# Black-Phoenix/CUDA-SfM

Measured on AMD Instinct MI355X. Metric: RANSAC E-matrix hypotheses/sec (8-point, fused scoring), inlier-mask parity vs CPU oracle, higher is better.
Workload: dtype f32

## Files before the change

cuda-sfm_amd/csrc/prefilter_lds.hpp:

```cpp
#pragma once
#include "prefilter_record.hpp"

namespace sfm {

constexpr int kPfTileMax = 1024;
constexpr int kPfWaves = 16;
constexpr int kPfRing = 128;

constexpr int kPfERow = 10;
constexpr int kPfWaveBytes = 32 * kPfERow * 4 + 32 * 4;
template <int RULE> struct PfLds {
    static constexpr int kFragsPerBlock = RULE == kPfRuleG ? 3 : 2;
    static constexpr int kBlockBytes = kFragsPerBlock * 64 * 16;
    static constexpr int kFrag = 0;
    static constexpr int kTileMax = kPfTileMax;
    int staged, pts, ring, wave, next, lut, bytes;
    __host__ __device__ explicit PfLds(int tile, int ring_entries = kPfRing, int entry_bytes = 8)
    {
        staged = (tile + 63) & ~63;
        pts = kFrag + (staged / 32) * kBlockBytes;
        ring = pts + staged * 16;
        ring = (ring + ring_entries * entry_bytes - 1) & ~(ring_entries * entry_bytes - 1);
        wave = ring + kPfWaves * ring_entries * entry_bytes;
        next = wave + kPfWaves * kPfWaveBytes;
        lut = next + 16;
        bytes = lut + 32;
    }
};
static_assert(kPfRing * 8 == 1024, "ring slots are addressed with (offset & 1023) | base");

static inline int pf_tile_points(int ld, int tmax)
{
    const int ntiles = (ld + tmax - 1) / tmax;
    const int t = ((ld + ntiles - 1) / ntiles + 31) & ~31;
    return t < 32 ? 32 : t;
}

constexpr unsigned long long kPfSumCountsMin = 1ull << 21;
static inline bool pf_sums_counts_at(unsigned count, int ld, int tile)
{
    return (unsigned long long)count * (unsigned long long)((ld + tile - 1) / tile) >= kPfSumCountsMin;
}

}
```

cuda-sfm_amd/csrc/prefilter_record.hpp:

```cpp
#pragma once
#include "prefilter_math.hpp"

namespace sfm {

typedef _Float16 h8 __attribute__((ext_vector_type(8)));

constexpr int kPfRuleG = 0, kPfRuleBand = 1, kPfRuleBandPack = 2, kPfRuleBandTile = 3;
constexpr uint32_t kPfTileFlagScan = 1u;
constexpr uint32_t kPfTileFlagBSafe = 2u;
constexpr int kPfGroup = 32;
constexpr unsigned short kPfFlagScan = 0x3C00u;

struct alignas(16) PfRecord {
    unsigned short lo[16];
    unsigned short hi[16];
};
static_assert(sizeof(PfRecord) == 64, "4 x 16 bytes per hypothesis");

#if defined(__HIPCC__)
__device__ __forceinline__ uint32_t pf_cells_slot(uint32_t key, uint32_t mask) { return (key >> 7) & mask; }

__device__ __forceinline__ void pf_prep_store(const float e[9], float thr, float B, const PfScales &sc, const uint32_t *__restrict__ cells,
                                              uint32_t cells_mask, PfRecord *out)
{
// ... 115 lines not shown
__device__ __forceinline__ uint32_t pf_tile_flags(const float e[9], float B, const uint32_t *__restrict__ cells, uint32_t cells_mask);
__device__ __forceinline__ uint4 pf_tile_record(const float e[9], float B, const uint32_t *__restrict__ cells, uint32_t cells_mask)
{
    float dn, lin;
    prefilter_band_hyp_terms(e, B, dn, lin);
    return make_uint4(pf_tile_flags(e, B, cells, cells_mask), __float_as_uint(dn), __float_as_uint(lin), 0u);
}

__device__ __forceinline__ uint32_t pf_tile_flags(const float e[9], float B, const uint32_t *__restrict__ cells, uint32_t cells_mask)
{
    const PfGrid grid = prefilter_grid(B);
    int cx0, cx1, cy0, cy1;
    const int zs = prefilter_zero_divisor_cells(e, B, grid, cx0, cx1, cy0, cy1);
    bool scan = zs == 2;
    if (zs == 1) scan = !cells || pf_cells_occupied(cells, cells_mask, cx0, cx1, cy0, cy1, 0);
    float et[9];
    prefilter_transposed(e, et);
    const int zb = prefilter_zero_divisor_cells(et, B, grid, cx0, cx1, cy0, cy1);
    bool b_safe = zb == 0;
    if (zb == 1) b_safe = cells && !pf_cells_occupied(cells, cells_mask, cx0, cx1, cy0, cy1, 1);
    return (scan ? kPfTileFlagScan : 0u) | (b_safe ? kPfTileFlagBSafe : 0u);
}

__device__ __forceinline__ void pf_tile_operands(const float e[9], uint32_t flags, float dn, float lin, float thr, float B, const PfBox &box, int half, h8 &n0, h8 &n1)
{
    const float d_mine = prefilter_band_divisor_max(e, lin, box, half);
    const float d_other = __shfl_xor(d_mine, 32);
    const float sigma = prefilter_band_sigma_from_maxima(dn, thr, B, half ? d_other : d_mine, half ? d_mine : d_other, (flags & kPfTileFlagBSafe) != 0u, kPfBandTopPack);
    _Float16 ns[kPfSlots];
    prefilter_band_hyp_slots(e, sigma, ns);
#pragma unroll
    for (int j = 0; j < 8; ++j) { n0[j] = half ? ns[8 + j] : ns[j]; n1[j] = half ? ns[24 + j] : ns[16 + j]; }
}

__device__ __forceinline__ void pf_band_record_expand(const uint4 r0, const uint4 r1, int half, h8 &n0, h8 &n1, uint32_t &flag)
{
    uint32_t o[8];
    if (half == 0) {
        const uint32_t A0 = r0.x, A1 = r0.y, A2 = r0.z, A3 = r0.w, A4 = r1.x, A5 = r1.y;
        o[0] = pf_pick(A0, 0, A0, 0); o[1] = pf_pick(A0, 1, A1, 0); o[2] = A1;                  o[3] = pf_pick(A2, 0, A2, 0);
        o[4] = pf_pick(A2, 1, A3, 0); o[5] = pf_pick(A3, 1, A3, 1); o[6] = A4;                  o[7] = pf_pick(A4, 1, A5, 0);
        flag = 0u;
    } else {
        const uint32_t B0 = r0.x, B1 = r0.y, B2 = r0.z, B3 = r0.w, B4 = r1.x;
        o[0] = B0;                  o[1] = pf_pick(B0, 1, B1, 0); o[2] = pf_pick(B1, 1, B1, 1); o[3] = B2;
        o[4] = B3;                  o[5] = (B4 & 0xFFFFu) | 0x3C000000u; o[6] = 0u;              o[7] = 0u;
        flag = B4 >> 16;
    }
    n0 = __builtin_bit_cast(h8, uint4{ o[0], o[1], o[2], o[3] });
    n1 = __builtin_bit_cast(h8, uint4{ o[4], o[5], o[6], o[7] });
}
#endif

}
```

cuda-sfm_amd/csrc/ransac_prefilter.hip:

```cpp
#include "ransac_device.hpp"
#include "block_ops.hpp"
#include "prefilter_math.hpp"
#include "prefilter_record.hpp"
#include "prefilter_lds.hpp"

namespace sfm {

typedef float f16v __attribute__((ext_vector_type(16)));


__device__ constexpr int kPfESlot[9] = { 2, 6, 1, 3, 5, 7, 0, 4, 8 };
__device__ __forceinline__ uint32_t shift_in_reject(uint32_t rejected, float nt, float G)
{
    return __builtin_amdgcn_alignbit(rejected, __float_as_uint(fmaf(-nt, nt, G)), 31);
}

__device__ __forceinline__ uint32_t scan16(const f16v &nt, const f16v &G)
{
    uint32_t rejected = 0u;
#pragma unroll
    for (int r = 0; r < 16; ++r) rejected = shift_in_reject(rejected, nt[r], G[r]);
    return rejected;
}

// ... 74 lines not shown

#define PF_SCHED_STEP()                                                 \
    do {                                                                \
        if (RULE != kPfRuleG) {                                         \
            __builtin_amdgcn_sched_group_barrier(0x008, 1, 0);          \
            __builtin_amdgcn_sched_group_barrier(0x002, 8, 0);          \
            __builtin_amdgcn_sched_group_barrier(0x008, 1, 0);          \
            __builtin_amdgcn_sched_group_barrier(0x002, 8, 0);          \
        } else {                                                        \
            __builtin_amdgcn_sched_group_barrier(0x008, 1, 0);          \
            __builtin_amdgcn_sched_group_barrier(0x002, 11, 0);         \
            __builtin_amdgcn_sched_group_barrier(0x008, 1, 0);          \
            __builtin_amdgcn_sched_group_barrier(0x002, 11, 0);         \
            __builtin_amdgcn_sched_group_barrier(0x008, 1, 0);          \
            __builtin_amdgcn_sched_group_barrier(0x002, 11, 0);         \
        }                                                               \
    } while (0)

constexpr int kPfVarTickets = 1;
constexpr int kPfVarDrainLocal = 2;
constexpr int kPfVarClosedDecode = 4;
constexpr int kPfVarAnswerEpilogue = 8;
constexpr int kPfVarDrainK1 = 16, kPfVarDrainK7 = 32;

constexpr int pf_score_waves_per_simd(int var, int rule, int fl2, int pipe, int wide, int prio)
{
    return ((var & kPfVarTickets) == 0 && (rule == kPfRuleBandTile || rule == kPfRuleBandPack) && !fl2 && !pipe && !wide && !prio) ? 5 : 4;
}

template <int W, int VAR = 0, int RULE = kPfRuleBandTile, int FL2 = 0, int PIPE = 0, int WIDE = 0, int PRIO = 0>
__global__ __launch_bounds__(W * 64, pf_score_waves_per_simd(VAR, RULE, FL2, PIPE, WIDE, PRIO))
void ransac_score_prefilter(const float *__restrict__ X0, const float *__restrict__ X1, int ld, int n,
                            const float *__restrict__ Ecand, const PfRecord *__restrict__ recs, uint32_t h0, uint32_t count, float thr,
                            int dynamic, int tile,
                            int *__restrict__ counts, uint32_t *__restrict__ tick,
                            unsigned long long *best_key, unsigned long long *best_key2, unsigned long long *__restrict__ clk,
                            const unsigned long long *__restrict__ bound_word, const uint32_t *__restrict__ tile_boxes)
{
    extern __shared__ __attribute__((aligned(16))) unsigned char smem[];
    const int lane = threadIdx.x & 63;
    const int wave = __builtin_amdgcn_readfirstlane(threadIdx.x >> 6);
    const bool probe = clk && blockIdx.x == 0 && blockIdx.y == 0 && threadIdx.x == 0;
    unsigned long long c0 = 0, w0 = 0;
    if (clk && blockIdx.x == 0 && blockIdx.y == 0 && wave == 0) { c0 = clock64(); w0 = wall_clock64(); }
#if SFM_AB
    const uint32_t trace_blk = blockIdx.y * gridDim.x + blockIdx.x;
    unsigned long long *trace = (clk && trace_blk < (uint32_t)kTraceBlocks) ? clk + 8 + (size_t)trace_blk * kTraceWords : nullptr;
    if (trace && threadIdx.x == 0) {
        trace[0] = wall_clock64();
        trace[2] = ((unsigned long long)__builtin_amdgcn_s_getreg((20 << 0) | (0 << 6) | (31 << 11)) << 32) |
                   (unsigned long long)__builtin_amdgcn_s_getreg((4 << 0) | (0 << 6) | (31 << 11));
        trace[3] = ((unsigned long long)blockIdx.y << 32) | blockIdx.x;
    }
#define PF_PHASE(k) do { if (probe1) clk[k] = wall_clock64() - w0; } while (0)
#else
#define PF_PHASE(k) do { } while (0)
#endif
    const int half = lane >> 5, row = lane & 31;
    const uint32_t npass = (count + (uint32_t)kPfGroup - 1u) / (uint32_t)kPfGroup;
    const uint32_t nstatic = gridDim.x * (uint32_t)W;
    using LT = PfLds<RULE>;
    constexpr bool kBand = RULE != kPfRuleG, kTile = RULE == kPfRuleBandTile, kPack = RULE == kPfRuleBandPack || kTile;
    static_assert(!(FL2 && kPack) && !((VAR & kPfVarTickets) && kPack), "the recorded variants were built on the v_alignbit scan");
    constexpr bool kTail9 = kPack && W == 16 && !FL2 && !PIPE && !WIDE && !PRIO && !(VAR & kPfVarTickets);
    static_assert(kTail9 || (VAR & ~kPfVarTickets) == 0, "the pass-tail switches belong to the product's two rules");
    constexpr int kDrainMore = !kTail9 ? 0 : (VAR & kPfVarDrainK1) ? 1 : (VAR & kPfVarDrainK7) ? 7 : (VAR & kPfVarDrainLocal) ? 3 : 0;
    constexpr bool kDecodeTable = !(kTail9 && (VAR & kPfVarClosedDecode));
    constexpr bool kSumCounts = kTail9 && !(VAR & kPfVarAnswerEpilogue);
    constexpr int kRing = FL2 ? 256 : kPfRing;
    constexpr int kEnt = WIDE ? 16 : 8;
    static_assert(!WIDE || (kPack && !PIPE && !FL2), "wide entries: the packed scan's plain loop only");
    const LT L(tile, kRing, kEnt);
    float *etab = reinterpret_cast<float *>(smem + L.wave + wave * kPfWaveBytes);
    int *cnt = reinterpret_cast<int *>(etab + 32 * kPfERow);

    PfFrags afrag = {};
    uint32_t key0 = 0u;
    float rec_dn = 0.0f, rec_lin = 0.0f;
    float e_row[9] = {};
    auto fetch_pass = [&](uint32_t pass, PfFrags &af, uint32_t &k0, float (&e)[9], float &dn, float &lin) {
        const uint32_t hf = pass * (uint32_t)kPfGroup;
        const uint32_t h = hf + (uint32_t)min(row, (int)min((uint32_t)kPfGroup, count - hf) - 1);
        if (kTile) {
            const float *src = Ecand + 9 * (size_t)h;
#pragma unroll
            for (int k = 0; k < 9; ++k) e[k] = src[k];
            const uint4 rec = reinterpret_cast<const uint4 *>(recs)[h];
            k0 = rec.x; dn = __uint_as_float(rec.y); lin = __uint_as_float(rec.z);
            return;
        }
        const uint4 *r = reinterpret_cast<const uint4 *>(recs + h) + 2 * half;
        const uint4 r0 = r[0], r1 = r[1];
        if (kBand) pf_band_record_expand(r0, r1, half, af.n0, af.n1, k0);
        else pf_record_expand(r0, r1, half, af.n0, af.n1, af.t, k0);
        if (half == 0) {
            const float *src = Ecand + 9 * (size_t)h;
#pragma unroll
            for (int k = 0; k < 9; ++k) e[k] = src[k];
        }
    };
    auto install_rows = [&](const float (&e)[9]) {
        if (half == 0) {
#pragma unroll
            for (int k = 0; k < 9; ++k) etab[32 * k + row] = e[kPfESlot[k]];
            cnt[row] = 0;
        }
    };
    uint32_t ps = blockIdx.x * (uint32_t)W + (uint32_t)wave;
    bool have = ps < npass;
    if (have) { fetch_pass(ps, afrag, key0, e_row, rec_dn, rec_lin); install_rows(e_row); }

    SFM_PHASE("stage_tile");
    uint32_t *next_idx = reinterpret_cast<uint32_t *>(smem + L.next);
    if (threadIdx.x == 0) *next_idx = (uint32_t)W;
    if (kPack && kDecodeTable && threadIdx.x < 32) smem[L.lut + threadIdx.x] = (unsigned char)pf_pack_code((int)threadIdx.x);
    float pf_B = 0.0f;
    uint32_t bw[8] = {};
    uint32_t bw_lane = 0u;
    if (kTile) {
        pf_B = __uint_as_float((uint32_t)(__hip_atomic_load(reinterpret_cast<const uint32_t *>(bound_word), __ATOMIC_RELAXED, __HIP_MEMORY_SCOPE_AGENT)));
        bw_lane = __hip_atomic_load(tile_boxes + 8 * blockIdx.y + (lane & 7), __ATOMIC_RELAXED, __HIP_MEMORY_SCOPE_AGENT);
    }
    __syncthreads();
    const int tile_first = blockIdx.y * tile;
    for (int t = threadIdx.x; t < L.staged; t += W * 64) {
        const int p = tile_first + t;
        float u = 0.f, v = 0.f, x = 0.f, y = 0.f;
        const bool real = p < n && t < tile;
// ... 14 lines not shown
#pragma unroll
            for (int hh = 0; hh < 2; ++hh) {
                h8 c;
#pragma unroll
                for (int j = 0; j < 8; ++j) c[j] = bn[ks * 16 + hh * 8 + j];
                *reinterpret_cast<h8 *>(blk + ks * 1024 + (hh * 32 + col) * 16) = c;
            }
        if (RULE == kPfRuleG) {
#pragma unroll
            for (int hh = 0; hh < 2; ++hh) {
                h8 c;
#pragma unroll
                for (int j = 0; j < 8; ++j) c[j] = bt[hh * 8 + j];
                *reinterpret_cast<h8 *>(blk + 2048 + (hh * 32 + col) * 16) = c;
            }
        }
    }
    __syncthreads();
    PfBox tbox = {};
    auto build_operands = [&](const float (&e)[9], uint32_t fl, float dn, float lin) {
        int half_l = half;
        float thr_l = thr, B_l = pf_B;
        asm volatile("" : "+v"(half_l), "+s"(thr_l), "+s"(B_l));
        pf_tile_operands(e, fl, dn, lin, thr_l, B_l, tbox, half_l, afrag.n0, afrag.n1);
        key0 = fl & kPfTileFlagScan;
    };
    if (kTile) {
#pragma unroll
        for (int k = 0; k < 8; ++k) bw[k] = (uint32_t)__builtin_amdgcn_readlane((int)bw_lane, k);
        pf_B = uniform(pf_B);
        tbox = pf_box_from_bits(bw, pf_B);
        tbox = PfBox{ uniform(tbox.xlo), uniform(tbox.xhi), uniform(tbox.ylo), uniform(tbox.yhi), uniform(tbox.ulo), uniform(tbox.uhi), uniform(tbox.vlo), uniform(tbox.vhi) };
        if (have) build_operands(e_row, key0, rec_dn, rec_lin);
    }
#if SFM_AB
    if (probe) clk[2] = wall_clock64() - w0;
#endif
    const int npb = (min(tile, ld - tile_first) + 31) >> 5;
    const int npp = (npb + 1) >> 1;
    const float4 *pts = reinterpret_cast<const float4 *>(smem + L.pts);
    lds_cf *etab_l = (lds_cf *)etab;
    lds_i *cnt_l = (lds_i *)cnt;
    lds_cu8 *lut_l = (lds_cu8 *)(smem + L.lut);
    const uint32_t ring_base = (uint32_t)(size_t)(__attribute__((address_space(3))) unsigned char *)(smem + L.ring) + (uint32_t)wave * (uint32_t)(kRing * kEnt);
    uint32_t ring_mask = (uint32_t)(kRing * kEnt - 1);
    asm("" : "+v"(ring_mask));
    auto ring_at = [&](uint32_t index8) {
        return (lds_u2 *)((__attribute__((address_space(3))) unsigned char *)0 + ((index8 & ring_mask) | ring_base));
    };
    auto ring_at16 = [&](uint32_t index16) {
        return (lds_u4 *)((__attribute__((address_space(3))) unsigned char *)0 + ((index16 & ring_mask) | ring_base));
    };
    lds_ch8 *frag_lane = (lds_ch8 *)(smem + LT::kFrag) + lane;
    const ThrBand band = make_band(thr);
    uint32_t passes_done = 0;

    while (have) {
        SFM_PHASE("pass_begin");
        const uint32_t h_first = ps * (uint32_t)kPfGroup;
        const int nvalid = (int)min((uint32_t)kPfGroup, count - h_first);
#if SFM_AB
        const bool probe1 = probe && passes_done == 0u;
#endif
        uint32_t ps_next = ps + nstatic;
        if (dynamic) {
            uint32_t got = 0u;
            if (lane == 0) got = atomicAdd(next_idx, 1u);
            got = (uint32_t)__builtin_amdgcn_readfirstlane((int)got);
            ps_next = (got / (uint32_t)W) * nstatic + blockIdx.x * (uint32_t)W + (got % (uint32_t)W);
        }
        {
            const bool scan = key0 != 0u;
            const unsigned long long sm = __ballot(scan);
            uint32_t todo = (uint32_t)sm | (uint32_t)(sm >> 32);
            uint32_t survive = 0u;
            while (todo) {
                const int r = __builtin_ctz(todo);
                todo &= todo - 1u;
                const float se[6] = { etab[6 * 32 + r], etab[2 * 32 + r], etab[r], etab[3 * 32 + r], etab[7 * 32 + r], etab[4 * 32 + r] };
                bool z = false;
                for (int j = 0; j < L.staged / 64; ++j) {
                    const float4 q = pts[j * 64 + lane];
                    z = z || prefilter_zero_divisor(se, q.x, q.z);
                }
                if (__ballot(z) != 0ull) survive |= 1u << r;
            }
            if (survive != 0u && ((survive >> row) & 1u)) {
                const h8 zero = {};
                afrag.n0 = zero; afrag.n1 = zero; afrag.t = zero;
                if (half) { afrag.n1[3] = (_Float16)1.0f; afrag.t[7] = (_Float16)0.0009765625f; }
            }
        }
        PF_PHASE(3);

        int head = 0, nq = 0;
        const uint32_t lane_tag = (uint32_t)(size_t)(lds_cf4 *)pts + (uint32_t)(row * 16) + (uint32_t)(half * 4);
        auto decide_first = [&](uint32_t &rest, uint32_t tag) {
            const int b = __builtin_clz(rest);
            rest &= ~(0x80000000u >> b);
            int hl, sub;
            if (kPack) {
                const uint32_t code = kDecodeTable ? (uint32_t)lut_l[b] : pf_pack_code_closed(b);
                hl = (int)(code & 31u) + (int)(tag & 4u); sub = (int)(code >> 5);
            } else {
                const int r = kBand ? b >> 1 : b & 15;
                sub = kBand ? b & 1 : b >> 4;
                hl = r + (r & 12) + (int)(tag & 4u);
            }
            if (hl < nvalid) {
                const f4v q = *(lds_cf4 *)((__attribute__((address_space(3))) const unsigned char *)0 + ((tag & ~15u) + ((uint32_t)sub << 9)));
                lds_cf *e = etab_l + hl;
                const v2f p0 = { e[0], e[32] }, p1 = { e[64], e[96] }, p2 = { e[128], e[160] }, p3 = { e[192], e[224] };
                const float e8 = e[256];
                if (pf_exact_inlier(p0, p1, p2, p3, e8, v2f{ q.x, q.y }, v2f{ q.z, q.w }, band))
                    __hip_atomic_fetch_add(cnt_l + hl, 1, __ATOMIC_RELAXED, __HIP_MEMORY_SCOPE_WORKGROUP);
            }
        };
        auto flush = [&](int m, auto more_c) {
            constexpr int kMore = decltype(more_c)::value;
            uint32_t rest = 0, tag = 0;
            if (PRIO == 2) __builtin_amdgcn_s_setprio(2);
            if (lane < m) {
                const u2v ent = *ring_at(((uint32_t)head + (uint32_t)lane) * 8u);
                tag = ent.y;
                rest = ent.x;
                decide_first(rest, tag);
                if constexpr (kMore > 0) {
#pragma unroll 1
                    for (int it = 0; it < kMore && rest != 0u; ++it) decide_first(rest, tag);
                }
            }
            const unsigned long long more = __ballot(rest != 0u);
            if (more) {
                const int slot = __builtin_amdgcn_mbcnt_hi((uint32_t)(more >> 32), __builtin_amdgcn_mbcnt_lo((uint32_t)more, 0u));
                if (rest) *ring_at(((uint32_t)(head + nq) + (uint32_t)slot) * 8u) = u2v{ rest, tag };
            }
            head = (head + m) & (kRing - 1);
            nq += __builtin_popcountll(more) - m;
// ... 40 lines not shown
            const f4v qA = *(lds_cf4 *)((__attribute__((address_space(3))) const unsigned char *)0 + ((entA.y & ~15u) + ((uint32_t)(bA & 1) << 9)));
            const f4v qB = *(lds_cf4 *)((__attribute__((address_space(3))) const unsigned char *)0 + ((entB.y & ~15u) + ((uint32_t)(bB & 1) << 9)));
            lds_cf *eA = etab_l + hcA, *eB = etab_l + hcB;
            const v2f a0 = { eA[0], eA[32] }, a1 = { eA[64], eA[96] }, a2 = { eA[128], eA[160] }, a3 = { eA[192], eA[224] };
            const float a8 = eA[256];
            const v2f b0 = { eB[0], eB[32] }, b1 = { eB[64], eB[96] }, b2 = { eB[128], eB[160] }, b3 = { eB[192], eB[224] };
            const float b8 = eB[256];
            const bool inA = pf_exact_inlier(a0, a1, a2, a3, a8, v2f{ qA.x, qA.y }, v2f{ qA.z, qA.w }, band);
            const bool inB = pf_exact_inlier(b0, b1, b2, b3, b8, v2f{ qB.x, qB.y }, v2f{ qB.z, qB.w }, band);
            if (inA && hlA < nvalid) __hip_atomic_fetch_add(cnt_l + hlA, 1, __ATOMIC_RELAXED, __HIP_MEMORY_SCOPE_WORKGROUP);
            if (inB && hlB < nvalid) __hip_atomic_fetch_add(cnt_l + hlB, 1, __ATOMIC_RELAXED, __HIP_MEMORY_SCOPE_WORKGROUP);
            const unsigned long long moreA = __ballot(restA != 0u), moreB = __ballot(restB != 0u);
            if (moreA | moreB) {
                const int nA = __builtin_popcountll(moreA);
                const int slotA = __builtin_amdgcn_mbcnt_hi((uint32_t)(moreA >> 32), __builtin_amdgcn_mbcnt_lo((uint32_t)moreA, 0u));
                const int slotB = nA + __builtin_amdgcn_mbcnt_hi((uint32_t)(moreB >> 32), __builtin_amdgcn_mbcnt_lo((uint32_t)moreB, 0u));
                if (restA) *ring_at(((uint32_t)(head + nq) + (uint32_t)slotA) * 8u) = u2v{ restA, entA.y };
                if (restB) *ring_at(((uint32_t)(head + nq) + (uint32_t)slotB) * 8u) = u2v{ restB, entB.y };
            }
            head = (head + 128) & (kRing - 1);
            nq += __builtin_popcountll(moreA) + __builtin_popcountll(moreB) - 128;
        };

        if constexpr (kPack && PIPE) {
        PfFrags fa = load_point_frags<RULE>(frag_lane, 0), fb = load_point_frags<RULE>(frag_lane, 1);
        lds_ch8 *fp = frag_lane + 2 * (LT::kBlockBytes / 16);
        const f16v zero16 = {};
        f16v a0, a1, b0, b1;
        a0 = __builtin_amdgcn_mfma_f32_32x32x16_f16(afrag.n0, fa.n0, zero16, 0, 0, 0);
        a1 = __builtin_amdgcn_mfma_f32_32x32x16_f16(afrag.n0, fb.n0, zero16, 0, 0, 0);
        a0 = __builtin_amdgcn_mfma_f32_32x32x16_f16(afrag.n1, fa.n1, a0, 0, 0, 0);
        a1 = __builtin_amdgcn_mfma_f32_32x32x16_f16(afrag.n1, fb.n1, a1, 0, 0, 0);
        fa = load_point_frags<RULE>(fp, 0);
        fb = load_point_frags<RULE>(fp, 1);
        fp += 2 * (LT::kBlockBytes / 16);
        auto phase = [&](const f16v &c0, const f16v &c1, f16v &m0, f16v &m1, int pp) {
            SFM_PHASE("scan_two_steps");
            __builtin_amdgcn_sched_barrier(0);
            m0 = __builtin_amdgcn_mfma_f32_32x32x16_f16(afrag.n0, fa.n0, zero16, 0, 0, 0);
            __builtin_amdgcn_sched_barrier(0);
            const u6v d = __builtin_amdgcn_cvt_scalef32_2xpk16_bf6_f32(c0, c1, 1.0f);
            __builtin_amdgcn_sched_barrier(0);
            m1 = __builtin_amdgcn_mfma_f32_32x32x16_f16(afrag.n0, fb.n0, zero16, 0, 0, 0);
            __builtin_amdgcn_sched_barrier(0);
            const uint32_t rej32 = pack_reject_bits(d);
            __builtin_amdgcn_sched_barrier(0);
// ... 85 lines not shown
            PF_SCHED_STEP();
            __builtin_amdgcn_sched_barrier(0);
            fb = load_point_frags<RULE>(fp, 1);
            fp += 2 * (LT::kBlockBytes / 16);
            __builtin_amdgcn_sched_barrier(0);
            mfma_step<RULE>(afrag, fa, g0, n0);
            const uint32_t rej_second = kBand ? scan16_band(n1) : scan16(n1, g1);
            PF_SCHED_STEP();
            __builtin_amdgcn_sched_barrier(0);
            const uint32_t rej32 = kBand ? (((rej_first << 1) & 0xAAAAAAAAu) | (rej_second & 0x55555555u))
                                                       : ((rej_first << 16) | rej_second);
            const bool mine = rej32 != 0xFFFFFFFFu;
            const unsigned long long any = __ballot(mine);
            SFM_PHASE("append_and_inloop_flush");
            if (any) {
                if (FL2) { while (nq >= 128) flush2(); }
                else
                while (nq >= 64) flush(64, kInLoop);
                const int slot = __builtin_amdgcn_mbcnt_hi((uint32_t)(any >> 32), __builtin_amdgcn_mbcnt_lo((uint32_t)any, 0u));
                if (mine) *ring_at(((uint32_t)(head + nq) + (uint32_t)slot) * 8u) = u2v{ ~rej32, lane_tag + ((uint32_t)pp << 10) };
                nq += __builtin_popcountll(any);
            }
        }
        }
        PF_PHASE(4);
        SFM_PHASE("pass_end_fetch_next");
        const bool have_next = ps_next < npass;
        PfFrags afrag_next = afrag;
        uint32_t key0n = 0u;
        float e_next[9] = {}, dn_next = 0.0f, lin_next = 0.0f;
        if (have_next) fetch_pass(ps_next, afrag_next, key0n, e_next, dn_next, lin_next);
        SFM_PHASE("drain_flush");
        if (FL2) { while (nq >= 128) flush2(); }
        if (WIDE) { while (nq > 0) flush_w(min(nq, 64)); }
        while (nq > 0) flush(min(nq, 64), kDrain);
        SFM_PHASE("epilogue");
        PF_PHASE(7);
        if (VAR & kPfVarTickets) {
        if (lane < nvalid) {
            const int c = cnt[lane];
            if (c) atomicAdd(&counts[h_first + lane], c);
        }
        asm volatile("s_waitcnt vmcnt(0)" ::: "memory");
        uint32_t t = 0;
        if (lane == 0) t = atomicAdd(&tick[ps], 1u);
        t = __builtin_amdgcn_readfirstlane(t);
        if (t == gridDim.y - 1) {
            unsigned long long k = 0;
            if (lane < nvalid) {
                const int c = __hip_atomic_load(&counts[h_first + lane], __ATOMIC_RELAXED, __HIP_MEMORY_SCOPE_AGENT);
                k = pack_key((uint32_t)c, h0 + h_first + (uint32_t)lane);
            }
            k = wave_max(k);
            if (lane == 0 && k) {
                atomicMax(best_key, k);
                if (best_key2) atomicMax(best_key2, k);
            }
        }
        } else if (kSumCounts) {
        if (lane < nvalid) {
            const int c = cnt[lane];
            if (c) __hip_atomic_fetch_add(&counts[h_first + lane], c, __ATOMIC_RELAXED, __HIP_MEMORY_SCOPE_AGENT);
        }
        if (have_next) {
            if (kTile) build_operands(e_next, key0n, dn_next, lin_next);
            else { afrag = afrag_next; key0 = key0n; }
            install_rows(e_next);
        }
        } else {
        uint32_t c_mine = 0u;
        unsigned long long old = 0ull;
        if (lane < nvalid) {
            c_mine = (uint32_t)cnt[lane];
            unsigned long long *acc = reinterpret_cast<unsigned long long *>(tick) + (h_first + (uint32_t)lane);
            old = atomicAdd(acc, (1ull << 32) | (unsigned long long)c_mine);
        }
        const int nvalid_done = nvalid;
        const uint32_t h_done = h_first;
        if (have_next) {
            if (kTile) build_operands(e_next, key0n, dn_next, lin_next);
            else { afrag = afrag_next; key0 = key0n; }
            install_rows(e_next);
        }
// ... 412 lines not shown
    }
    pair->pf_seen_epoch = pair->bound_epoch;
    pair->pf_rule = rule;
    return rule;
}

bool prefilter_usable(const sfm_pair *pair, const sfm_ransac_params &p, uint32_t count)
{
    PfScales sc;
    return pair->state.unit_z && pair->state.have_bound && count >= 16384u && (uint64_t)count * (uint64_t)pair->ld >= (1ull << 27) && prefilter_scales(p.threshold, sc);
}

static int pf_tile_of(const sfm_pair *pair, const sfm_ransac_params &p)
{
    if (SFM_SW(p, 1) == 7 && pair->pf_rule == kPfRuleBand) return pf_tile_points(pair->ld, 1536);
    return pf_tile_points(pair->ld, kPfTileMax);
}

int prefilter_tile_points(const sfm_pair *pair, const sfm_ransac_params &p) { return pf_tile_of(pair, p); }

static int pf_tail_var(const sfm_pair *pair, const sfm_ransac_params &p, uint32_t count)
{
    const bool large = pf_sums_counts_at(count, pair->ld, pf_tile_of(pair, p));
    if (pair->pf_rule == kPfRuleBandTile && SFM_SW(p, 1) == 16) return kPfVarDrainK1;
    if (pair->pf_rule == kPfRuleBandTile && SFM_SW(p, 1) == 17) return kPfVarDrainK7;
    int var = 0;
    const bool lab = SFM_SW(p, 3) >= 8 && SFM_SW(p, 3) < 16;
    if (lab && (SFM_SW(p, 3) & 1)) var |= kPfVarDrainLocal;
    if (lab && (SFM_SW(p, 3) & 2)) var |= kPfVarClosedDecode;
    const bool sum = (lab && (SFM_SW(p, 3) & 4)) ? false : (large || (SFM_SW(p, 1) >= 16 && SFM_SW(p, 1) <= 18));
    if (!sum) var |= kPfVarAnswerEpilogue;
    return var;
}

bool prefilter_sums_counts(const sfm_pair *pair, const sfm_ransac_params &p, uint32_t count)
{
    const bool product_rule = pair->pf_rule == kPfRuleBandTile || pair->pf_rule == kPfRuleBandPack;
    const bool variant = SFM_SW(p, 1) == 5 || (SFM_SW(p, 1) >= 11 && SFM_SW(p, 1) <= 15);
    return product_rule && !variant && !(pf_tail_var(pair, p, count) & kPfVarAnswerEpilogue);
}

int launch_score_prefilter(sfm_pair *pair, ShardSlot &s, hipStream_t stream, const sfm_ransac_params &p, uint32_t h0, uint32_t count, unsigned long long *key2)
{
    sfm_ctx *ctx = pair->ctx;
    PfScales sc;
    if (!prefilter_scales(p.threshold, sc)) { set_error("threshold %g outside the pre-filter's range", (double)p.threshold); return SFM_E_INVALID; }
    const int waves = (SFM_SW(p, 1) == 5 || SFM_SW(p, 1) == 12) ? 12 : kPfWaves;
    const int tile = pf_tile_of(pair, p);
    const int ntiles = (pair->ld + tile - 1) / tile;
    const uint32_t npass = (count + (uint32_t)kPfGroup - 1u) / (uint32_t)kPfGroup;
    const uint32_t iters = (npass + (uint32_t)waves - 1) / (uint32_t)waves;
    uint32_t cols = (uint32_t)ctx->num_cus / (uint32_t)ntiles;
    if (SFM_SW(p, 2) > 0) cols = (uint32_t)SFM_SW(p, 2);
    if (cols > iters) cols = iters;
    if (cols < 1) cols = 1;
    const int dynamic = SFM_SW(p, 1) == 2 ? 0 : 1;
    const int var = SFM_SW(p, 3) >= 16 ? SFM_SW(p, 3) - 16 : 0;
    const int rule = pair->pf_rule;
    const int tail_var = pf_tail_var(pair, p, count);
    const bool fl2 = rule == kPfRuleBand && waves == kPfWaves && SFM_SW(p, 1) == 9;
    const bool wide = rule == kPfRuleBandTile && SFM_SW(p, 1) == 13;
    const int lds_bytes = wide ? PfLds<kPfRuleBand>(tile, kPfRing, 16).bytes : fl2 ? PfLds<kPfRuleBand>(tile, 256).bytes : rule != kPfRuleG ? PfLds<kPfRuleBand>(tile).bytes : PfLds<kPfRuleG>(tile).bytes;
    if (lds_bytes > 160 * 1024) { set_error("pre-filter tile of %d points needs %d bytes of LDS", tile, lds_bytes); return SFM_E_INVALID; }
    auto launch = [&](auto kernel) -> int {
        const int rc_lds = allow_big_lds(ctx, reinterpret_cast<const void *>(kernel));
        if (rc_lds != SFM_OK) return rc_lds;
        const float *x0 = rule == kPfRuleBandTile ? reinterpret_cast<const float *>(pair->d_pts4s) : pair->d_X[0];
        hipLaunchKernelGGL(kernel, dim3(cols, ntiles), dim3(waves * 64), lds_bytes, stream,
                           x0, pair->d_X[1], pair->ld, pair->n, s.Ecand, reinterpret_cast<const PfRecord *>(s.pf), h0, count, p.threshold,
                           dynamic, tile, s.counts, s.tick, s.key, key2, pair->d_clk, pair->d_bound, pair->d_tile_boxes);
        return SFM_OK;
    };
    int rcl;
#if SFM_AB
    if (rule == kPfRuleG && waves == 12) rcl = launch(&ransac_score_prefilter<12, 0, kPfRuleG>);
    else if (rule == kPfRuleG && var == 1) rcl = launch(&ransac_score_prefilter<16, 1, kPfRuleG>);
    else if (rule == kPfRuleG) rcl = launch(&ransac_score_prefilter<16, 0, kPfRuleG>);
    else if (waves == 12) rcl = launch(&ransac_score_prefilter<12, 0, kPfRuleBand>);
    else if (fl2) rcl = launch(&ransac_score_prefilter<16, 0, kPfRuleBand, 1>);
    else if (rule == kPfRuleBand) rcl = launch(&ransac_score_prefilter<16, 0, kPfRuleBand>);
    else if (SFM_SW(p, 1) == 11) rcl = launch(&ransac_score_prefilter<16, 0, kPfRuleBandPack, 0, 1>);
    else if (SFM_SW(p, 1) == 12) rcl = launch(&ransac_score_prefilter<12, 0, kPfRuleBandPack, 0, 1>);
    else if (wide) rcl = launch(&ransac_score_prefilter<16, 0, kPfRuleBandTile, 0, 0, 1>);
    else if (rule == kPfRuleBandTile && SFM_SW(p, 1) == 14) rcl = launch(&ransac_score_prefilter<16, 0, kPfRuleBandTile, 0, 0, 0, 1>);
    else if (rule == kPfRuleBandTile && SFM_SW(p, 1) == 15) rcl = launch(&ransac_score_prefilter<16, 0, kPfRuleBandTile, 0, 0, 0, 2>);
    else if (tail_var != 0 && tail_var != kPfVarAnswerEpilogue) {
        rcl = SFM_E_INVALID;
#define PF_TAIL_CASE(V) case V: rcl = rule == kPfRuleBandPack ? launch(&ransac_score_prefilter<16, V, kPfRuleBandPack>) : launch(&ransac_score_prefilter<16, V, kPfRuleBandTile>); break
        switch (tail_var) {
        PF_TAIL_CASE(2); PF_TAIL_CASE(4); PF_TAIL_CASE(6); PF_TAIL_CASE(10); PF_TAIL_CASE(12); PF_TAIL_CASE(14);
        case kPfVarDrainK1: rcl = launch(&ransac_score_prefilter<16, kPfVarDrainK1, kPfRuleBandTile>); break;
        case kPfVarDrainK7: rcl = launch(&ransac_score_prefilter<16, kPfVarDrainK7, kPfRuleBandTile>); break;
        default: set_error("pass-tail switches %d: no such instance", tail_var); break;
        }
#undef PF_TAIL_CASE
    }
    else
#endif
    if (tail_var & kPfVarAnswerEpilogue) rcl = rule == kPfRuleBandPack ? launch(&ransac_score_prefilter<16, kPfVarAnswerEpilogue, kPfRuleBandPack>)
                                                                       : launch(&ransac_score_prefilter<16, kPfVarAnswerEpilogue, kPfRuleBandTile>);
    else if (rule == kPfRuleBandPack) rcl = launch(&ransac_score_prefilter<16, 0, kPfRuleBandPack>);
    else rcl = launch(&ransac_score_prefilter<16, 0, kPfRuleBandTile>);
    (void)var; (void)fl2; (void)wide; (void)tail_var;
    if (rcl != SFM_OK) return rcl;
    SFM_HIP_TRY(hipGetLastError());
    pair->last_grid = (int)cols * ntiles; pair->last_block = waves * 64; pair->last_lds = lds_bytes;
    return SFM_OK;
}

}
```

profiles/ab_two_trees.py:

```python
import json
import os
import subprocess
import sys

ROOT = os.path.dirname(os.path.dirname(os.path.abspath(__file__)))
TREES = (("parent", os.path.abspath(sys.argv[1])), ("this", ROOT))
REPS = int(sys.argv[2]) if len(sys.argv) > 2 else 5
OUT = sys.argv[3] if len(sys.argv) > 3 else None
PROGRAMS = (("bench_headline", ["bench.py"]), ("bench_c4", ["bench.py", "--config", "c4"]), ("enqueue_probe", ["profiles/enqueue_probe.py"]))
KEEP = ("ms_per_step", "value", "unit", "hypotheses", "pipelined_enqueue_us_per_step", "pipelined_total_us_per_step",
        "serial_enqueue_us_per_step", "serial_total_us_per_step")

out = open(OUT, "w") if OUT else None
for name, cmd in PROGRAMS:
    for rep in range(REPS):
        for tree, path in TREES:
            r = subprocess.run(["timeout", "-k", "10", "240", sys.executable] + cmd, cwd=path, capture_output=True, text=True)
            lines = [ln for ln in r.stdout.splitlines() if ln.startswith("{")]
            for ln in lines:
                rec = json.loads(ln)
                msg = json.dumps({"program": name, "rep": rep, "tree": tree, **{k: rec[k] for k in KEEP if k in rec}})
                print(msg, flush=True)
                if out:
                    out.write(msg + "\n"); out.flush()
            if r.returncode != 0 or not lines:
                print("FAILED", name, tree, r.returncode, r.stdout[-1500:], r.stderr[-3000:], flush=True)
                sys.exit(1)
```

profiles/trace_probe.py:

```python
import json, os, sys
import numpy as np
sys.path.insert(0, os.path.dirname(os.path.dirname(os.path.abspath(__file__))))
import torch
import cuda_sfm_amd_ab as S
from cuda_sfm_amd_ab import synth

dev = torch.device("cuda", 0)
ctx = S.Context(0, torch.cuda.current_stream().cuda_stream)
cases = [(4096, int(h)) for h in sys.argv[1:]] or [(4096, 1 << 20), (4096, 131072), (16384, 1 << 20)]
for n, H in cases:
    scene = synth.two_view_scene(n)
    d_sift = torch.from_numpy(scene["sift"].view(np.uint8).reshape(n, 576)).to(dev)
    pair = S.ImagePair(ctx, scene["K"], scene["Kinv"], 2, n)
    pair.fillXU(d_sift)
    p = S.default_params(n, num_hypotheses=H, kernel=S.KERNEL_PREFILTER)
    for _ in range(10):
        pair.ransac_score(p)
    torch.cuda.synchronize()
    t = pair.last_trace().astype(np.float64)
    us = 0.01
    start, wave_end = t[:, 0] * us, t[:, 4:20] * us
    t0 = start.min()
    start -= t0; wave_end -= t0
    blk_end = wave_end.max(axis=1)
    life = blk_end - start
    span = blk_end.max()
    xcc = (t[:, 2].astype(np.uint64) >> np.uint64(32)).astype(int) & 0xF
    spread = wave_end.max(axis=1) - wave_end.min(axis=1)
    live = (wave_end - start[:, None]).sum() / (span * len(t))
    out = {"matches": n, "hypotheses": H, "blocks": len(t), "span_us": round(span, 1), "last_start_us": round(float(start.max()), 1),
           "block_lifetime_us_p0_10_50_90_100": [round(float(x), 1) for x in np.percentile(life, [0, 10, 50, 90, 100])],
           "block_end_us_p10_50_90": [round(float(x), 1) for x in np.percentile(blk_end, [10, 50, 90])],
           "wave_end_spread_in_block_us_p50_90_100": [round(float(x), 1) for x in np.percentile(spread, [50, 90, 100])],
           "mean_live_waves_per_block_over_span": round(float(live), 2),
           "lifetime_by_xcc_us": {int(x): round(float(life[xcc == x].mean()), 1) for x in sorted(set(xcc))},
           "blocks_by_xcc": {int(x): int((xcc == x).sum()) for x in sorted(set(xcc))}}
    print(json.dumps(out), flush=True)
    pair.close()
```

Measured before the change: 2.739 billion.

## Pair two 32-hypothesis groups per wave unit to amortize per-pass tile work

New measurement: 2.833 billion (median of 6 runs). 1.03x the previous value.

```diff
diff --git a/cuda-sfm_amd/csrc/prefilter_lds.hpp b/cuda-sfm_amd/csrc/prefilter_lds.hpp
--- a/cuda-sfm_amd/csrc/prefilter_lds.hpp
+++ b/cuda-sfm_amd/csrc/prefilter_lds.hpp
@@ -8,21 +8,22 @@
 constexpr int kPfRing = 128;
 
 constexpr int kPfERow = 10;
-constexpr int kPfWaveBytes = 32 * kPfERow * 4 + 32 * 4;
+constexpr int kPfPassRows = 32, kPfPairRows = 64;
+constexpr int pf_wave_bytes(int rows) { return rows * kPfERow * 4 + rows * 4; }
 template <int RULE> struct PfLds {
     static constexpr int kFragsPerBlock = RULE == kPfRuleG ? 3 : 2;
     static constexpr int kBlockBytes = kFragsPerBlock * 64 * 16;
     static constexpr int kFrag = 0;
     static constexpr int kTileMax = kPfTileMax;
     int staged, pts, ring, wave, next, lut, bytes;
-    __host__ __device__ explicit PfLds(int tile, int ring_entries = kPfRing, int entry_bytes = 8)
+    __host__ __device__ explicit PfLds(int tile, int ring_entries = kPfRing, int entry_bytes = 8, int rows = RULE == kPfRuleG ? kPfPassRows : kPfPairRows)
     {
         staged = (tile + 63) & ~63;
         pts = kFrag + (staged / 32) * kBlockBytes;
         ring = pts + staged * 16;
         ring = (ring + ring_entries * entry_bytes - 1) & ~(ring_entries * entry_bytes - 1);
         wave = ring + kPfWaves * ring_entries * entry_bytes;
-        next = wave + kPfWaves * kPfWaveBytes;
+        next = wave + kPfWaves * pf_wave_bytes(rows);
         lut = next + 16;
         bytes = lut + 32;
     }
@@ -42,4 +43,10 @@
     return (unsigned long long)count * (unsigned long long)((ld + tile - 1) / tile) >= kPfSumCountsMin;
 }
 
+constexpr unsigned long long kPfPairPassesMin = 1ull << 22;
+static inline bool pf_pairs_passes_at(unsigned count, int ld, int tile)
+{
+    return (unsigned long long)count * (unsigned long long)((ld + tile - 1) / tile) >= kPfPairPassesMin;
 }
+
+}
diff --git a/cuda-sfm_amd/csrc/prefilter_record.hpp b/cuda-sfm_amd/csrc/prefilter_record.hpp
--- a/cuda-sfm_amd/csrc/prefilter_record.hpp
+++ b/cuda-sfm_amd/csrc/prefilter_record.hpp
@@ -161,15 +161,33 @@
     return (scan ? kPfTileFlagScan : 0u) | (b_safe ? kPfTileFlagBSafe : 0u);
 }
 
-__device__ __forceinline__ void pf_tile_operands(const float e[9], uint32_t flags, float dn, float lin, float thr, float B, const PfBox &box, int half, h8 &n0, h8 &n1)
-{
-    const float d_mine = prefilter_band_divisor_max(e, lin, box, half);
-    const float d_other = __shfl_xor(d_mine, 32);
+#endif
+
+SFM_HD void pf_tile_operands_half(const float e[9], uint32_t flags, float dn, float thr, float B, int half, float d_mine, float d_other, h8 &n0, h8 &n1)
+{
     const float sigma = prefilter_band_sigma_from_maxima(dn, thr, B, half ? d_other : d_mine, half ? d_mine : d_other, (flags & kPfTileFlagBSafe) != 0u, kPfBandTopPack);
     _Float16 ns[kPfSlots];
     prefilter_band_hyp_slots(e, sigma, ns);
 #pragma unroll
     for (int j = 0; j < 8; ++j) { n0[j] = half ? ns[8 + j] : ns[j]; n1[j] = half ? ns[24 + j] : ns[16 + j]; }
+}
+
+SFM_HD void pf_tile_operands_full(const float e[9], uint32_t flags, float dn, float lin, float thr, float B, const PfBox &box, h8 &x0, h8 &y0, h8 &x1, h8 &y1)
+{
+    const float Da = prefilter_band_divisor_max(e, lin, box, 0), Db = prefilter_band_divisor_max(e, lin, box, 1);
+    const float sigma = prefilter_band_sigma_from_maxima(dn, thr, B, Da, Db, (flags & kPfTileFlagBSafe) != 0u, kPfBandTopPack);
+    _Float16 ns[kPfSlots];
+    prefilter_band_hyp_slots(e, sigma, ns);
+#pragma unroll
+    for (int j = 0; j < 8; ++j) { x0[j] = ns[j]; y0[j] = ns[8 + j]; x1[j] = ns[16 + j]; y1[j] = ns[24 + j]; }
+}
+
+#if defined(__HIPCC__)
+__device__ __forceinline__ void pf_tile_operands(const float e[9], uint32_t flags, float dn, float lin, float thr, float B, const PfBox &box, int half, h8 &n0, h8 &n1)
+{
+    const float d_mine = prefilter_band_divisor_max(e, lin, box, half);
+    const float d_other = __shfl_xor(d_mine, 32);
+    pf_tile_operands_half(e, flags, dn, thr, B, half, d_mine, d_other, n0, n1);
 }
 
 __device__ __forceinline__ void pf_band_record_expand(const uint4 r0, const uint4 r1, int half, h8 &n0, h8 &n1, uint32_t &flag)
diff --git a/cuda-sfm_amd/csrc/ransac_prefilter.hip b/cuda-sfm_amd/csrc/ransac_prefilter.hip
--- a/cuda-sfm_amd/csrc/ransac_prefilter.hip
+++ b/cuda-sfm_amd/csrc/ransac_prefilter.hip
@@ -120,9 +120,11 @@
 constexpr int kPfVarClosedDecode = 4;
 constexpr int kPfVarAnswerEpilogue = 8;
 constexpr int kPfVarDrainK1 = 16, kPfVarDrainK7 = 32;
+constexpr int kPfVarSinglePass = 64;
 
 constexpr int pf_score_waves_per_simd(int var, int rule, int fl2, int pipe, int wide, int prio)
 {
+    if (var == 0 && rule == kPfRuleBandTile && !fl2 && !pipe && !wide && !prio) return 4;
     return ((var & kPfVarTickets) == 0 && (rule == kPfRuleBandTile || rule == kPfRuleBandPack) && !fl2 && !pipe && !wide && !prio) ? 5 : 4;
 }
 
@@ -155,30 +157,35 @@
 #define PF_PHASE(k) do { } while (0)
 #endif
     const int half = lane >> 5, row = lane & 31;
-    const uint32_t npass = (count + (uint32_t)kPfGroup - 1u) / (uint32_t)kPfGroup;
+    uint32_t npass = (count + (uint32_t)kPfGroup - 1u) / (uint32_t)kPfGroup;
     const uint32_t nstatic = gridDim.x * (uint32_t)W;
     using LT = PfLds<RULE>;
     constexpr bool kBand = RULE != kPfRuleG, kTile = RULE == kPfRuleBandTile, kPack = RULE == kPfRuleBandPack || kTile;
     static_assert(!(FL2 && kPack) && !((VAR & kPfVarTickets) && kPack), "the recorded variants were built on the v_alignbit scan");
     constexpr bool kTail9 = kPack && W == 16 && !FL2 && !PIPE && !WIDE && !PRIO && !(VAR & kPfVarTickets);
     static_assert(kTail9 || (VAR & ~kPfVarTickets) == 0, "the pass-tail switches belong to the product's two rules");
+    static_assert(!(VAR & kPfVarSinglePass) || (kTile && VAR == kPfVarSinglePass), "single passes: the per-tile rule's summing instance");
+    constexpr bool kPair = kTile && kTail9 && VAR == 0;
+    constexpr int kRows = kPair ? kPfPairRows : kPfPassRows, kUnit = kRows;
     constexpr int kDrainMore = !kTail9 ? 0 : (VAR & kPfVarDrainK1) ? 1 : (VAR & kPfVarDrainK7) ? 7 : (VAR & kPfVarDrainLocal) ? 3 : 0;
     constexpr bool kDecodeTable = !(kTail9 && (VAR & kPfVarClosedDecode));
     constexpr bool kSumCounts = kTail9 && !(VAR & kPfVarAnswerEpilogue);
     constexpr int kRing = FL2 ? 256 : kPfRing;
     constexpr int kEnt = WIDE ? 16 : 8;
     static_assert(!WIDE || (kPack && !PIPE && !FL2), "wide entries: the packed scan's plain loop only");
-    const LT L(tile, kRing, kEnt);
-    float *etab = reinterpret_cast<float *>(smem + L.wave + wave * kPfWaveBytes);
-    int *cnt = reinterpret_cast<int *>(etab + 32 * kPfERow);
+    if (kPair) npass = (npass + 1u) >> 1;
+    const LT L(tile, kRing, kEnt, kRows);
+    float *etab = reinterpret_cast<float *>(smem + L.wave + wave * pf_wave_bytes(kRows));
+    int *cnt = reinterpret_cast<int *>(etab + kRows * kPfERow);
 
     PfFrags afrag = {};
+    h8 bfrag_n0 = {}, bfrag_n1 = {};
     uint32_t key0 = 0u;
     float rec_dn = 0.0f, rec_lin = 0.0f;
     float e_row[9] = {};
     auto fetch_pass = [&](uint32_t pass, PfFrags &af, uint32_t &k0, float (&e)[9], float &dn, float &lin) {
-        const uint32_t hf = pass * (uint32_t)kPfGroup;
-        const uint32_t h = hf + (uint32_t)min(row, (int)min((uint32_t)kPfGroup, count - hf) - 1);
+        const uint32_t hf = pass * (uint32_t)kUnit;
+        const uint32_t h = hf + (uint32_t)min(kPair ? lane : row, (int)min((uint32_t)kUnit, count - hf) - 1);
         if (kTile) {
             const float *src = Ecand + 9 * (size_t)h;
 #pragma unroll
@@ -198,10 +205,11 @@
         }
     };
     auto install_rows = [&](const float (&e)[9]) {
-        if (half == 0) {
-#pragma unroll
-            for (int k = 0; k < 9; ++k) etab[32 * k + row] = e[kPfESlot[k]];
-            cnt[row] = 0;
+        if (kPair || half == 0) {
+            const int r = kPair ? lane : row;
+#pragma unroll
+            for (int k = 0; k < 9; ++k) etab[kRows * k + r] = e[kPfESlot[k]];
+            cnt[r] = 0;
         }
     };
     uint32_t ps = blockIdx.x * (uint32_t)W + (uint32_t)wave;
@@ -262,8 +270,21 @@
         int half_l = half;
         float thr_l = thr, B_l = pf_B;
         asm volatile("" : "+v"(half_l), "+s"(thr_l), "+s"(B_l));
+        key0 = fl & kPfTileFlagScan;
+        if constexpr (kPair) {
+            h8 x0, y0, x1, y1;
+            pf_tile_operands_full(e, fl, dn, lin, thr_l, B_l, tbox, x0, y0, x1, y1);
+            u4v xa = __builtin_bit_cast(u4v, x0), ya = __builtin_bit_cast(u4v, y0), xb = __builtin_bit_cast(u4v, x1), yb = __builtin_bit_cast(u4v, y1);
+#pragma unroll
+            for (int w = 0; w < 4; ++w) {
+                const u2v sa = __builtin_amdgcn_permlane32_swap(xa[w], ya[w], false, false);
+                const u2v sb = __builtin_amdgcn_permlane32_swap(xb[w], yb[w], false, false);
+                xa[w] = sa.x; ya[w] = sa.y; xb[w] = sb.x; yb[w] = sb.y;
+            }
+            afrag.n0 = __builtin_bit_cast(h8, xa); afrag.n1 = __builtin_bit_cast(h8, xb);
+            bfrag_n0 = __builtin_bit_cast(h8, ya); bfrag_n1 = __builtin_bit_cast(h8, yb);
+        } else
         pf_tile_operands(e, fl, dn, lin, thr_l, B_l, tbox, half_l, afrag.n0, afrag.n1);
-        key0 = fl & kPfTileFlagScan;
     };
     if (kTile) {
 #pragma unroll
@@ -297,8 +318,10 @@
 
     while (have) {
         SFM_PHASE("pass_begin");
-        const uint32_t h_first = ps * (uint32_t)kPfGroup;
-        const int nvalid = (int)min((uint32_t)kPfGroup, count - h_first);
+        const uint32_t h_first = ps * (uint32_t)kUnit;
+        const int nvalid_unit = (int)min((uint32_t)kUnit, count - h_first);
+        int nvalid = min(nvalid_unit, kPfGroup), hoff = 0;
+        const int nscan = (kPair && nvalid_unit > kPfGroup) ? 2 : 1;
 #if SFM_AB
         const bool probe1 = probe && passes_done == 0u;
 #endif
@@ -309,31 +332,29 @@
             got = (uint32_t)__builtin_amdgcn_readfirstlane((int)got);
             ps_next = (got / (uint32_t)W) * nstatic + blockIdx.x * (uint32_t)W + (got % (uint32_t)W);
         }
-        {
-            const bool scan = key0 != 0u;
-            const unsigned long long sm = __ballot(scan);
-            uint32_t todo = (uint32_t)sm | (uint32_t)(sm >> 32);
+        const unsigned long long scan_rows = __ballot(key0 != 0u);
+        int head = 0, nq = 0;
+        auto patch_zero_divisor_rows = [&](int sc) {
+            uint32_t todo = kPair ? (uint32_t)(sc ? scan_rows >> 32 : scan_rows) : ((uint32_t)scan_rows | (uint32_t)(scan_rows >> 32));
             uint32_t survive = 0u;
             while (todo) {
-                const int r = __builtin_ctz(todo);
+                const int r = __builtin_ctz(todo) + hoff;
                 todo &= todo - 1u;
-                const float se[6] = { etab[6 * 32 + r], etab[2 * 32 + r], etab[r], etab[3 * 32 + r], etab[7 * 32 + r], etab[4 * 32 + r] };
+                const float se[6] = { etab[6 * kRows + r], etab[2 * kRows + r], etab[r], etab[3 * kRows + r], etab[7 * kRows + r], etab[4 * kRows + r] };
                 bool z = false;
                 for (int j = 0; j < L.staged / 64; ++j) {
                     const float4 q = pts[j * 64 + lane];
                     z = z || prefilter_zero_divisor(se, q.x, q.z);
                 }
-                if (__ballot(z) != 0ull) survive |= 1u << r;
+                if (__ballot(z) != 0ull) survive |= 1u << (r - hoff);
             }
             if (survive != 0u && ((survive >> row) & 1u)) {
                 const h8 zero = {};
                 afrag.n0 = zero; afrag.n1 = zero; afrag.t = zero;
                 if (half) { afrag.n1[3] = (_Float16)1.0f; afrag.t[7] = (_Float16)0.0009765625f; }
             }
-        }
-        PF_PHASE(3);
-
-        int head = 0, nq = 0;
+        };
+
         const uint32_t lane_tag = (uint32_t)(size_t)(lds_cf4 *)pts + (uint32_t)(row * 16) + (uint32_t)(half * 4);
         auto decide_first = [&](uint32_t &rest, uint32_t tag) {
             const int b = __builtin_clz(rest);
@@ -349,11 +370,11 @@
             }
             if (hl < nvalid) {
                 const f4v q = *(lds_cf4 *)((__attribute__((address_space(3))) const unsigned char *)0 + ((tag & ~15u) + ((uint32_t)sub << 9)));
-                lds_cf *e = etab_l + hl;
-                const v2f p0 = { e[0], e[32] }, p1 = { e[64], e[96] }, p2 = { e[128], e[160] }, p3 = { e[192], e[224] };
-                const float e8 = e[256];
+                lds_cf *e = etab_l + hl + hoff;
+                const v2f p0 = { e[0], e[kRows] }, p1 = { e[2 * kRows], e[3 * kRows] }, p2 = { e[4 * kRows], e[5 * kRows] }, p3 = { e[6 * kRows], e[7 * kRows] };
+                const float e8 = e[8 * kRows];
                 if (pf_exact_inlier(p0, p1, p2, p3, e8, v2f{ q.x, q.y }, v2f{ q.z, q.w }, band))
-                    __hip_atomic_fetch_add(cnt_l + hl, 1, __ATOMIC_RELAXED, __HIP_MEMORY_SCOPE_WORKGROUP);
+                    __hip_atomic_fetch_add(cnt_l + hl + hoff, 1, __ATOMIC_RELAXED, __HIP_MEMORY_SCOPE_WORKGROUP);
             }
         };
         auto flush = [&](int m, auto more_c) {
@@ -440,6 +461,9 @@
             nq += __builtin_popcountll(moreA) + __builtin_popcountll(moreB) - 128;
         };
 
+        for (int sc = 0; ; ++sc) {
+        patch_zero_divisor_rows(sc);
+        PF_PHASE(3);
         if constexpr (kPack && PIPE) {
         PfFrags fa = load_point_frags<RULE>(frag_lane, 0), fb = load_point_frags<RULE>(frag_lane, 1);
         lds_ch8 *fp = frag_lane + 2 * (LT::kBlockBytes / 16);
@@ -571,6 +595,11 @@
                 nq += __builtin_popcountll(any);
             }
         }
+        }
+        if (sc + 1 >= nscan) break;
+        while (nq > 0) flush(min(nq, 64), kDrain);
+        afrag.n0 = bfrag_n0; afrag.n1 = bfrag_n1;
+        hoff = kPfGroup; nvalid = nvalid_unit - kPfGroup;
         }
         PF_PHASE(4);
         SFM_PHASE("pass_end_fetch_next");
@@ -607,7 +636,7 @@
             }
         }
         } else if (kSumCounts) {
-        if (lane < nvalid) {
+        if (lane < nvalid_unit) {
             const int c = cnt[lane];
             if (c) __hip_atomic_fetch_add(&counts[h_first + lane], c, __ATOMIC_RELAXED, __HIP_MEMORY_SCOPE_AGENT);
         }
@@ -1066,6 +1095,8 @@
 static int pf_tail_var(const sfm_pair *pair, const sfm_ransac_params &p, uint32_t count)
 {
     const bool large = pf_sums_counts_at(count, pair->ld, pf_tile_of(pair, p));
+    if (SFM_SW(p, 1) == 19) return 0;
+    if (SFM_SW(p, 1) == 20) return pair->pf_rule == kPfRuleBandTile ? kPfVarSinglePass : 0;
     if (pair->pf_rule == kPfRuleBandTile && SFM_SW(p, 1) == 16) return kPfVarDrainK1;
     if (pair->pf_rule == kPfRuleBandTile && SFM_SW(p, 1) == 17) return kPfVarDrainK7;
     int var = 0;
@@ -1074,6 +1105,7 @@
     if (lab && (SFM_SW(p, 3) & 2)) var |= kPfVarClosedDecode;
     const bool sum = (lab && (SFM_SW(p, 3) & 4)) ? false : (large || (SFM_SW(p, 1) >= 16 && SFM_SW(p, 1) <= 18));
     if (!sum) var |= kPfVarAnswerEpilogue;
+    if (var == 0 && pair->pf_rule == kPfRuleBandTile && !pf_pairs_passes_at(count, pair->ld, pf_tile_of(pair, p))) var = kPfVarSinglePass;
     return var;
 }
 
@@ -1093,18 +1125,21 @@
     const int tile = pf_tile_of(pair, p);
     const int ntiles = (pair->ld + tile - 1) / tile;
     const uint32_t npass = (count + (uint32_t)kPfGroup - 1u) / (uint32_t)kPfGroup;
-    const uint32_t iters = (npass + (uint32_t)waves - 1) / (uint32_t)waves;
+    const int rule = pair->pf_rule;
+    const int tail_var = pf_tail_var(pair, p, count);
+    const bool wide = rule == kPfRuleBandTile && SFM_SW(p, 1) == 13;
+    const bool paired_units = rule == kPfRuleBandTile && tail_var == 0 && waves == kPfWaves && !wide && SFM_SW(p, 1) != 14 && SFM_SW(p, 1) != 15;
+    const uint32_t nunits = paired_units ? (npass + 1u) / 2u : npass;
+    const uint32_t iters = (nunits + (uint32_t)waves - 1) / (uint32_t)waves;
     uint32_t cols = (uint32_t)ctx->num_cus / (uint32_t)ntiles;
     if (SFM_SW(p, 2) > 0) cols = (uint32_t)SFM_SW(p, 2);
     if (cols > iters) cols = iters;
     if (cols < 1) cols = 1;
     const int dynamic = SFM_SW(p, 1) == 2 ? 0 : 1;
     const int var = SFM_SW(p, 3) >= 16 ? SFM_SW(p, 3) - 16 : 0;
-    const int rule = pair->pf_rule;
-    const int tail_var = pf_tail_var(pair, p, count);
     const bool fl2 = rule == kPfRuleBand && waves == kPfWaves && SFM_SW(p, 1) == 9;
-    const bool wide = rule == kPfRuleBandTile && SFM_SW(p, 1) == 13;
-    const int lds_bytes = wide ? PfLds<kPfRuleBand>(tile, kPfRing, 16).bytes : fl2 ? PfLds<kPfRuleBand>(tile, 256).bytes : rule != kPfRuleG ? PfLds<kPfRuleBand>(tile).bytes : PfLds<kPfRuleG>(tile).bytes;
+    const int lds_bytes = wide ? PfLds<kPfRuleBand>(tile, kPfRing, 16, kPfPassRows).bytes : fl2 ? PfLds<kPfRuleBand>(tile, 256, 8, kPfPassRows).bytes
+                        : rule != kPfRuleG ? PfLds<kPfRuleBand>(tile, kPfRing, 8, paired_units ? kPfPairRows : kPfPassRows).bytes : PfLds<kPfRuleG>(tile).bytes;
     if (lds_bytes > 160 * 1024) { set_error("pre-filter tile of %d points needs %d bytes of LDS", tile, lds_bytes); return SFM_E_INVALID; }
     auto launch = [&](auto kernel) -> int {
         const int rc_lds = allow_big_lds(ctx, reinterpret_cast<const void *>(kernel));
@@ -1128,7 +1163,7 @@
     else if (wide) rcl = launch(&ransac_score_prefilter<16, 0, kPfRuleBandTile, 0, 0, 1>);
     else if (rule == kPfRuleBandTile && SFM_SW(p, 1) == 14) rcl = launch(&ransac_score_prefilter<16, 0, kPfRuleBandTile, 0, 0, 0, 1>);
     else if (rule == kPfRuleBandTile && SFM_SW(p, 1) == 15) rcl = launch(&ransac_score_prefilter<16, 0, kPfRuleBandTile, 0, 0, 0, 2>);
-    else if (tail_var != 0 && tail_var != kPfVarAnswerEpilogue) {
+    else if (tail_var != 0 && tail_var != kPfVarAnswerEpilogue && tail_var != kPfVarSinglePass) {
         rcl = SFM_E_INVALID;
 #define PF_TAIL_CASE(V) case V: rcl = rule == kPfRuleBandPack ? launch(&ransac_score_prefilter<16, V, kPfRuleBandPack>) : launch(&ransac_score_prefilter<16, V, kPfRuleBandTile>); break
         switch (tail_var) {
@@ -1144,6 +1179,7 @@
     if (tail_var & kPfVarAnswerEpilogue) rcl = rule == kPfRuleBandPack ? launch(&ransac_score_prefilter<16, kPfVarAnswerEpilogue, kPfRuleBandPack>)
                                                                        : launch(&ransac_score_prefilter<16, kPfVarAnswerEpilogue, kPfRuleBandTile>);
     else if (rule == kPfRuleBandPack) rcl = launch(&ransac_score_prefilter<16, 0, kPfRuleBandPack>);
+    else if (tail_var == kPfVarSinglePass) rcl = launch(&ransac_score_prefilter<16, kPfVarSinglePass, kPfRuleBandTile>);
     else rcl = launch(&ransac_score_prefilter<16, 0, kPfRuleBandTile>);
     (void)var; (void)fl2; (void)wide; (void)tail_var;
     if (rcl != SFM_OK) return rcl;
diff --git a/profiles/ab_two_trees.py b/profiles/ab_two_trees.py
--- a/profiles/ab_two_trees.py
+++ b/profiles/ab_two_trees.py
@@ -7,9 +7,12 @@
 TREES = (("parent", os.path.abspath(sys.argv[1])), ("this", ROOT))
 REPS = int(sys.argv[2]) if len(sys.argv) > 2 else 5
 OUT = sys.argv[3] if len(sys.argv) > 3 else None
-PROGRAMS = (("bench_headline", ["bench.py"]), ("bench_c4", ["bench.py", "--config", "c4"]), ("enqueue_probe", ["profiles/enqueue_probe.py"]))
-KEEP = ("ms_per_step", "value", "unit", "hypotheses", "pipelined_enqueue_us_per_step", "pipelined_total_us_per_step",
+PROGRAMS = (("bench_headline", ["bench.py"]), ("bench_c4", ["bench.py", "--config", "c4"]), ("enqueue_probe", ["profiles/enqueue_probe.py"]),
+            ("bench_c3", ["bench.py", "--config", "c3"]), ("bench_h524288", ["bench.py", "--hyps", "524288"]), ("bench_h131072", ["bench.py", "--hyps", "131072"]),
+            ("bench_serial", ["bench.py", "--serial"]))
+KEEP = ("ms_per_step", "serial_ms_per_step", "value", "unit", "hypotheses", "pipelined_enqueue_us_per_step", "pipelined_total_us_per_step",
         "serial_enqueue_us_per_step", "serial_total_us_per_step")
+PROGRAMS = tuple(pr for pr in PROGRAMS if pr[0] in sys.argv[4].split(",")) if len(sys.argv) > 4 else PROGRAMS[:3]
 
 out = open(OUT, "w") if OUT else None
 for name, cmd in PROGRAMS:
diff --git a/profiles/trace_probe.py b/profiles/trace_probe.py
--- a/profiles/trace_probe.py
+++ b/profiles/trace_probe.py
@@ -7,6 +7,8 @@
 
 dev = torch.device("cuda", 0)
 ctx = S.Context(0, torch.cuda.current_stream().cuda_stream)
+SW1 = [int(a[6:]) for a in sys.argv[1:] if a.startswith("--sw1=")]
+sys.argv = [a for a in sys.argv if not a.startswith("--sw1=")]
 cases = [(4096, int(h)) for h in sys.argv[1:]] or [(4096, 1 << 20), (4096, 131072), (16384, 1 << 20)]
 for n, H in cases:
     scene = synth.two_view_scene(n)
@@ -14,6 +16,8 @@
     pair = S.ImagePair(ctx, scene["K"], scene["Kinv"], 2, n)
     pair.fillXU(d_sift)
     p = S.default_params(n, num_hypotheses=H, kernel=S.KERNEL_PREFILTER)
+    if SW1:
+        p.reserved[1] = SW1[0]
     for _ in range(10):
         pair.ransac_score(p)
     torch.cuda.synchronize()
@@ -28,7 +32,7 @@
     xcc = (t[:, 2].astype(np.uint64) >> np.uint64(32)).astype(int) & 0xF
     spread = wave_end.max(axis=1) - wave_end.min(axis=1)
     live = (wave_end - start[:, None]).sum() / (span * len(t))
-    out = {"matches": n, "hypotheses": H, "blocks": len(t), "span_us": round(span, 1), "last_start_us": round(float(start.max()), 1),
+    out = {"sw1": SW1[0] if SW1 else 0, "matches": n, "hypotheses": H, "blocks": len(t), "span_us": round(span, 1), "last_start_us": round(float(start.max()), 1),
            "block_lifetime_us_p0_10_50_90_100": [round(float(x), 1) for x in np.percentile(life, [0, 10, 50, 90, 100])],
            "block_end_us_p10_50_90": [round(float(x), 1) for x in np.percentile(blk_end, [10, 50, 90])],
            "wave_end_spread_in_block_us_p50_90_100": [round(float(x), 1) for x in np.percentile(spread, [50, 90, 100])],
```
